# fixie-ai/ultravox

Measured on NVIDIA H100. Metric: audio-sec/s prefill (Llama-3.1-8B, 30s clip) at 1/2/4/8 H100; TTFT p50, higher is better.
Workload: dtype bf16

## Files before the change

include/uvx.h:

```cpp
#ifndef UVX_H_
#define UVX_H_

#include <stddef.h>
#include <stdint.h>

#ifdef __cplusplus
extern "C" {
#endif

#define UVX_ABI_VERSION 1

#define UVX_OK 0
#define UVX_ERR_ARG (-1)
#define UVX_ERR_CUDA (-2)
#define UVX_ERR_WS (-3)

typedef void* uvx_stream_t;

int uvx_abi_version(void);
const char* uvx_last_error(void);
int64_t uvx_launch_count(void);

size_t uvx_logmel_workspace(int64_t B, int64_t L, int n_mels);
int uvx_logmel(const float* wave, int64_t B, int64_t L, int n_mels, float* out_f32, void* out_tm,
               void* workspace, size_t workspace_bytes, uvx_stream_t stream);

int uvx_debug_mel_filters(int n_mels, float* host_dense);

int uvx_mel_to_timemajor(const float* mel, int64_t N, int n_mels, int64_t T, void* out_tm, uvx_stream_t stream);

enum { UVX_ACT_NONE = 0, UVX_ACT_GELU = 1, UVX_ACT_SWIGLU = 2 };
enum { UVX_DT_BF16 = 0, UVX_DT_F32 = 1 };
enum { UVX_TILE_PLAIN = 0, UVX_TILE_ROPE_PAIRS = 1, UVX_TILE_GATE_UP_8 = 8, UVX_TILE_GATE_UP_16 = 16 };

typedef struct uvx_gemm_args {
  const void* A;
  int64_t a_batch, a_rows, K;
  int64_t a_row_stride, a_batch_stride;
  const void* W;
  int64_t N, w_row_stride;
  void* C;
  int64_t c_row_stride, c_batch_rows, c_row_offset;
  const int32_t* c_row_map;
  const void* bias;
  const void* R;
  int64_t r_row_stride, r_batch_stride;
  float alpha;
  int32_t act;
  int32_t out_dtype;
  void* workspace;
  int64_t workspace_bytes;
  const void* norm_w;
  void* norm_out;
  float norm_eps;
  int32_t w_tiled;
  int32_t rope_cols;
  const float* rope_cos;
  const float* rope_sin;
  const int32_t* rope_positions;
  int64_t rope_rows_per_seq, rope_pos_offset;
  int32_t flags;
  int32_t w_perm;
} uvx_gemm_args;

int uvx_gemm_bf16(const uvx_gemm_args* args, uvx_stream_t stream);
int uvx_debug_gemm_override(int cfg, int splits);
int uvx_debug_gemm_stages(int n);
int uvx_debug_gemm_ws(int enable, int mode, int grid);
int uvx_debug_gemm_tma_store(int on);
int uvx_debug_gemm_times(void* dev_buf);
int uvx_debug_gemm_pf(int pf);
int uvx_debug_gemm_ws_times(void* dev_buf);
int uvx_tile_weight(const void* W, int64_t N, int64_t K, int64_t w_row_stride, int32_t R, int32_t interleave, void* out,
                    uvx_stream_t stream);
int uvx_debug_gemm_cluster(int cm, int cn);
int uvx_debug_gemm_mode(int mode);

int uvx_layernorm(const void* x, const void* w, const void* b, void* y, int64_t rows, int64_t cols,
                  int64_t x_row_stride, float eps, uvx_stream_t stream);
int uvx_rmsnorm(const void* x, const void* w, void* y, int64_t rows, int64_t cols, int64_t x_row_stride,
                int64_t group_rows, int64_t group_stride, int64_t valid_elems, float eps, uvx_stream_t stream);

typedef struct uvx_attn_args {
  const void *q, *k, *v;
  void* o;
  int64_t B, Hq, Hkv, Sq, Skv, D;
  int64_t q_rs, q_bs, k_rs, k_bs, v_rs, v_bs, o_rs, o_bs;
  const int32_t* kv_len;
  int32_t causal;
  int32_t block;
// ... 89 lines not shown
```

ultravox_b200/_lib.py:

```python
from __future__ import annotations

import ctypes as C
import os
import pathlib

_HERE = pathlib.Path(__file__).resolve().parent
LIB_PATH = _HERE / "libuvx.so"

c_i64, c_i32, c_f32, c_vp, c_sz = C.c_int64, C.c_int32, C.c_float, C.c_void_p, C.c_size_t


class GemmArgs(C.Structure):
    _fields_ = [("A", c_vp), ("a_batch", c_i64), ("a_rows", c_i64), ("K", c_i64), ("a_row_stride", c_i64),
                ("a_batch_stride", c_i64), ("W", c_vp), ("N", c_i64), ("w_row_stride", c_i64), ("C", c_vp),
                ("c_row_stride", c_i64), ("c_batch_rows", c_i64), ("c_row_offset", c_i64), ("c_row_map", c_vp),
                ("bias", c_vp), ("R", c_vp), ("r_row_stride", c_i64), ("r_batch_stride", c_i64), ("alpha", c_f32),
                ("act", c_i32), ("out_dtype", c_i32), ("workspace", c_vp), ("workspace_bytes", c_i64),
                ("norm_w", c_vp), ("norm_out", c_vp), ("norm_eps", c_f32), ("w_tiled", c_i32), ("rope_cols", c_i32),
                ("rope_cos", c_vp), ("rope_sin", c_vp), ("rope_positions", c_vp), ("rope_rows_per_seq", c_i64),
                ("rope_pos_offset", c_i64), ("flags", c_i32), ("w_perm", c_i32)]


class AttnArgs(C.Structure):
    _fields_ = [("q", c_vp), ("k", c_vp), ("v", c_vp), ("o", c_vp), ("B", c_i64), ("Hq", c_i64), ("Hkv", c_i64),
                ("Sq", c_i64), ("Skv", c_i64), ("D", c_i64), ("q_rs", c_i64), ("q_bs", c_i64), ("k_rs", c_i64),
                ("k_bs", c_i64), ("v_rs", c_i64), ("v_bs", c_i64), ("o_rs", c_i64), ("o_bs", c_i64), ("kv_len", c_vp),
                ("causal", c_i32), ("block", c_i32), ("scale", c_f32), ("lse", c_vp), ("kv_start", c_vp)]


SIGNATURES = {
    "uvx_abi_version": (C.c_int, []),
    "uvx_last_error": (C.c_char_p, []),
    "uvx_launch_count": (c_i64, []),
    "uvx_logmel_workspace": (c_sz, [c_i64, c_i64, C.c_int]),
    "uvx_logmel": (C.c_int, [c_vp, c_i64, c_i64, C.c_int, c_vp, c_vp, c_vp, c_sz, c_vp]),
    "uvx_debug_mel_filters": (C.c_int, [C.c_int, c_vp]),
    "uvx_mel_to_timemajor": (C.c_int, [c_vp, c_i64, C.c_int, c_i64, c_vp, c_vp]),
    "uvx_gemm_bf16": (C.c_int, [C.POINTER(GemmArgs), c_vp]),
    "uvx_debug_gemm_override": (C.c_int, [C.c_int, C.c_int]),
    "uvx_debug_gemm_cluster": (C.c_int, [C.c_int, C.c_int]),
    "uvx_debug_gemm_mode": (C.c_int, [C.c_int]),
    "uvx_debug_gemm_pf": (C.c_int, [C.c_int]),
    "uvx_debug_gemm_stages": (C.c_int, [C.c_int]),
    "uvx_debug_gemm_times": (C.c_int, [c_vp]),
    "uvx_debug_gemm_tma_store": (C.c_int, [C.c_int]),
    "uvx_debug_gemm_ws": (C.c_int, [C.c_int, C.c_int, C.c_int]),
    "uvx_debug_gemm_ws_times": (C.c_int, [C.c_void_p]),
    "uvx_tile_weight": (C.c_int, [c_vp, c_i64, c_i64, c_i64, c_i32, c_i32, c_vp, c_vp]),
    "uvx_layernorm": (C.c_int, [c_vp, c_vp, c_vp, c_vp, c_i64, c_i64, c_i64, c_f32, c_vp]),
    "uvx_rmsnorm": (C.c_int, [c_vp, c_vp, c_vp, c_i64, c_i64, c_i64, c_i64, c_i64, c_i64, c_f32, c_vp]),
    "uvx_attention": (C.c_int, [C.POINTER(AttnArgs), c_vp]),
    "uvx_debug_attn_tc": (C.c_int, [C.c_int]),
    "uvx_attention_enc_tc": (C.c_int, [c_vp, c_i64, c_i64, c_i64, c_i64, c_i64, c_i64, c_i64, c_vp, c_i64, c_vp, c_i32, c_f32, c_vp]),
    "uvx_rope": (C.c_int, [c_vp, c_i64, c_i64, C.c_int, C.c_int, C.c_int, c_vp, c_vp, c_vp, c_i64, c_i64, c_vp]),
    "uvx_swiglu": (C.c_int, [c_vp, c_vp, c_i64, c_i64, c_i64, C.c_int, c_vp]),
    "uvx_splice_plan": (C.c_int, [c_vp, c_vp, c_vp, c_i64, c_i64, c_i64, c_i64, c_vp, c_vp]),
    "uvx_embed_splice": (C.c_int, [c_vp, c_vp, c_i64, c_vp, c_vp, c_i64, c_i64, c_vp, c_vp]),
    "uvx_lm_head": (C.c_int, [c_vp, c_i64, c_i64, c_vp, c_i64, c_i64, c_vp, c_vp]),
    "uvx_gemv_bf16": (C.c_int, [c_vp, c_i64, c_i64, c_vp, c_i64, c_i64, c_i64, c_vp, c_i64, c_vp, c_i64, C.c_int, c_vp]),
    "uvx_kv_append": (C.c_int, [c_vp, c_i64, c_i64, c_i64, c_i64, c_vp, c_vp, c_i64, c_vp, c_i64, c_vp]),
    "uvx_gemv_fused_bf16": (C.c_int, [c_vp, c_i64, c_i64, c_vp, c_i64, c_i64, c_i64, c_vp, c_i64, c_vp, c_i64, C.c_int, c_vp, C.c_float,
                                      C.c_int, c_vp]),
    "uvx_rope_kv_append": (C.c_int, [c_vp, c_i64, c_i64, C.c_int, C.c_int, C.c_int, c_vp, c_vp, c_vp, c_vp, c_vp, c_i64, c_vp, c_vp]),
    "uvx_add_i32": (C.c_int, [c_vp, c_vp, c_i64, c_i32, c_vp]),
    "uvx_kv_write": (C.c_int, [c_vp, c_i64, c_i64, c_i64, c_i64, c_vp, c_vp, c_i64, c_i64, c_i64, c_i64, c_vp]),
    "uvx_repetition_penalty": (C.c_int, [c_vp, c_i64, c_i64, c_vp, c_i64, c_vp, c_f32, c_vp, c_vp]),
# ... 55 lines not shown
```

ultravox_b200/csrc/gemm_tc.cu:

```cuda
#include <stdlib.h>

#include "uvx_common.cuh"
#include "tc_ptx.cuh"

namespace uvx {

struct GemmParams {
  int64_t a_rows, a_batch, K, N;
  void* C;
  int64_t c_row_stride, c_batch_rows, c_row_offset;
  const int32_t* c_row_map;
  const bf16* bias;
  const bf16* R;
  int64_t r_row_stride, r_batch_stride;
  float alpha;
  int act, out_f32;
  int m_tiles;
  int n_tiles, num_tiles;
  int splits, kb_per_split;
  float* ws_partial;
  const bf16* norm_w;
  bf16* norm_out;
  float norm_eps;
  int w_tiled;
  int w_perm;
  int swiglu;
  const float* rope_cos;
  const float* rope_sin;
  const int32_t* rope_pos;
  int64_t rope_rows_per_seq, rope_pos_offset;
  int rope_cols;
  int stages;
  int cm, cn;
};

static constexpr int kSmemTotal = 227 * 1024;
static constexpr int kMaxStages = 8;
static constexpr int kGemmThreads = 384;

template <int MT, int BN>
struct WgLayout {
  static constexpr int kABytes = MT * 128 * kBK * 2;
  static constexpr int kWBytes = BN * kBK * 2;
  static constexpr int kStageBytes = kABytes + kWBytes;
  static constexpr int kRingMax = kSmemTotal - 1024 - 256;
  static constexpr int kStages = kRingMax / kStageBytes > kMaxStages ? kMaxStages : kRingMax / kStageBytes;
  static constexpr int kAcc = BN / 2;
  static_assert(kStages >= 2, "ring too shallow");
  static_assert(MT * kAcc <= 128, "accumulators must fit the register file");
};

__device__ __forceinline__ int tile_col(int tc, int perm) {
  if (!perm) return tc;
  const int q = tc >> 5, j = tc & 31;
  return j < 16 ? 16 * q + j : 64 + 16 * q + (j - 16);
}

__device__ __forceinline__ int64_t out_row(const GemmParams& p, int b, int64_t m) {
  return p.c_row_map ? (int64_t)p.c_row_map[(int64_t)b * p.a_rows + m] : (int64_t)b * p.c_batch_rows + m + p.c_row_offset;
}

template <int BN, int I>
__device__ __forceinline__ void swiglu_row(const GemmParams& p, const float* a, int h, int cq, bf16* crow, int64_t n_out0) {
#pragma unroll
  for (int j = 0; j < BN / 8; ++j) {
    if ((8 * j) % (2 * I) >= I) continue;
    const int64_t f = n_out0 + (8 * j / (2 * I)) * I + (8 * j) % (2 * I) + cq;
    if (f >= p.N / 2) continue;
// ... 6 lines not shown
      o[e] = __bfloat162float(__float2bfloat16_rn(silu_fast(gate))) * up;
    }
    *reinterpret_cast<__nv_bfloat162*>(crow + f) = __floats2bfloat162_rn(o[0], o[1]);
  }
}

__device__ __forceinline__ void rope_store(const GemmParams& p, float x1a, float x1b, float x2a, float x2b, int64_t pos, int d, bf16* crow) {
  const float2 cs = *reinterpret_cast<const float2*>(p.rope_cos + pos * 64 + d);
  const float2 sn = *reinterpret_cast<const float2*>(p.rope_sin + pos * 64 + d);
  float o1a, o2a, o1b, o2b;
  rope_pair(__bfloat162float(__float2bfloat16_rn(x1a * p.alpha)), __bfloat162float(__float2bfloat16_rn(x2a * p.alpha)), cs.x, sn.x, o1a, o2a);
  rope_pair(__bfloat162float(__float2bfloat16_rn(x1b * p.alpha)), __bfloat162float(__float2bfloat16_rn(x2b * p.alpha)), cs.y, sn.y, o1b, o2b);
  *reinterpret_cast<__nv_bfloat162*>(crow + d) = __floats2bfloat162_rn(o1a, o1b);
  *reinterpret_cast<__nv_bfloat162*>(crow + d + 64) = __floats2bfloat162_rn(o2a, o2b);
}

template <int MT, int BN>
__global__ void __launch_bounds__(kGemmThreads, 1)
gemm_wg_kernel(const __grid_constant__ CUtensorMap tmA, const __grid_constant__ CUtensorMap tmW, const GemmParams p) {
  using L = WgLayout<MT, BN>;
  pdl_trigger();
  extern __shared__ uint8_t smem_raw[];
  uint8_t* smem = (uint8_t*)(((uintptr_t)smem_raw + 1023) & ~(uintptr_t)1023);
  uint64_t* full_bar = (uint64_t*)(smem + p.stages * L::kStageBytes);
  uint64_t* empty_bar = full_bar + kMaxStages;

  const int wg = threadIdx.x >> 7, tid = threadIdx.x & 127;
  const int tiles_m_total = p.m_tiles * (int)p.a_batch;
  const int num_kb = (int)((p.K + kBK - 1) / kBK);
  const int stages = p.stages;
  const int csize = p.cm * p.cn;
  const int rank = csize > 1 ? (int)cluster_ctarank() : 0;
  const int rm = rank / p.cn, rn = rank % p.cn;
  const int cluster_tiles_m = tiles_m_total / p.cm;
  const int num_units = p.num_tiles / csize * p.splits;
  const int first_unit = blockIdx.x / csize, unit_step = gridDim.x / csize;

  if (threadIdx.x == 0) {
    for (int s = 0; s < stages; ++s) {
      mbar_init(&full_bar[s], 1);
      mbar_init(&empty_bar[s], 8 * csize);
    }
    asm volatile("fence.mbarrier_init.release.cluster;" ::: "memory");
    asm volatile("fence.proxy.async.shared::cta;" ::: "memory");
  }
  if (csize > 1) cluster_sync();
  else __syncthreads();
  pdl_wait();

  if (wg == 0) {
    asm volatile("setmaxnreg.dec.sync.aligned.u32 40;");
    if (tid == 0) {
      asm volatile("prefetch.tensormap [%0];" ::"l"(&tmA) : "memory");
      asm volatile("prefetch.tensormap [%0];" ::"l"(&tmW) : "memory");
      const int a_slice = MT * 128 / p.cn, w_slice = BN / p.cm;
      const uint16_t row_mask = (uint16_t)(((1u << p.cn) - 1u) << (rm * p.cn));
      uint16_t col_mask = 0;
      for (int j = 0; j < p.cm; ++j) col_mask |= (uint16_t)(1u << (j * p.cn + rn));
      int s = 0;
      uint32_t ph = 0;
      for (int unit = first_unit; unit < num_units; unit += unit_step) {
        const int ctile = unit / p.splits, split = unit % p.splits;
        const int tm_idx = (ctile % cluster_tiles_m) * p.cm + rm;
        const int tn_idx = (ctile / cluster_tiles_m) * p.cn + rn;
        const int b = tm_idx / p.m_tiles;
        const int m0 = (tm_idx % p.m_tiles) * (MT * 128);
        const int kb_begin = split * p.kb_per_split;
        const int kb_end = min(num_kb, kb_begin + p.kb_per_split);
        const int wt_base = tn_idx * num_kb * BN;
        for (int kb = kb_begin; kb < kb_end; ++kb) {
          mbar_wait(&empty_bar[s], ph ^ 1u);
          uint8_t* sa = smem + s * L::kStageBytes;
          mbar_expect_tx(&full_bar[s], (uint32_t)L::kStageBytes);
          uint8_t* da = sa + rn * a_slice * (kBK * 2);
          if (p.cn > 1) tma_load_3d_mc(da, &tmA, kb * kBK, m0 + rn * a_slice, b, &full_bar[s], row_mask);
          else tma_load_3d(da, &tmA, kb * kBK, m0, b, &full_bar[s]);
          uint8_t* dw = sa + L::kABytes + rm * w_slice * (kBK * 2);
          const int w0 = p.w_tiled ? 0 : kb * kBK;
          const int w1 = (p.w_tiled ? wt_base + kb * BN : tn_idx * BN) + rm * w_slice;
          if (p.cm > 1) tma_load_2d_mc(dw, &tmW, w0, w1, &full_bar[s], col_mask);
          else tma_load_2d(dw, &tmW, w0, w1, &full_bar[s]);
          if (++s == stages) { s = 0; ph ^= 1u; }
        }
      }
    }
    if (csize > 1) cluster_sync();
    return;
  }

  asm volatile("setmaxnreg.inc.sync.aligned.u32 232;");
  const int c = wg - 1;
  const int warp = tid >> 5, lane = tid & 31;
  auto release = [&](int slot) {
    __syncwarp();
    if (csize == 1) {
      if (lane == 0) mbar_arrive(&empty_bar[slot]);
    } else if (lane < csize) {
      mbar_arrive_cluster(&empty_bar[slot], (uint32_t)lane);
    }
  };
  int s = 0;
  uint32_t ph = 0;
  for (int unit = first_unit; unit < num_units; unit += unit_step) {
    const int ctile = unit / p.splits, split = unit % p.splits;
    const int tm_idx = (ctile % cluster_tiles_m) * p.cm + rm;
    const int tn_idx = (ctile / cluster_tiles_m) * p.cn + rn;
    const int b = tm_idx / p.m_tiles;
    const int m0 = (tm_idx % p.m_tiles) * (MT * 128);
    const int n0 = tn_idx * BN;
    const int kb_begin = split * p.kb_per_split;
    const int kb_end = min(num_kb, kb_begin + p.kb_per_split);

    float acc[MT][L::kAcc];
    int prev = -1;
    for (int kb = kb_begin; kb < kb_end; ++kb) {
      mbar_wait(&full_bar[s], ph);
      const uint32_t sa = smem_u32(smem + s * L::kStageBytes);
      const uint64_t dw = make_wgmma_desc(sa + L::kABytes);
      wgmma_fence();
#pragma unroll
      for (int mt = 0; mt < MT; ++mt) {
        const uint64_t da = make_wgmma_desc(sa + (mt * 128 + c * 64) * (kBK * 2));
#pragma unroll
        for (int k = 0; k < kBK / 16; ++k)
          Wgmma<BN>::mma(acc[mt], da + (uint64_t)(2 * k), dw + (uint64_t)(2 * k), (kb > kb_begin || k > 0) ? 1u : 0u);
      }
      wgmma_commit();
      wgmma_wait<1>();
      if (prev >= 0) release(prev);
      prev = s;
      if (++s == stages) { s = 0; ph ^= 1u; }
    }
    wgmma_wait<0>();
    release(prev);

    const int rq = warp * 16 + (lane >> 2);
    const int cq = 2 * (lane & 3);
    if (p.splits > 1) {
      float* part = p.ws_partial + (size_t)split * (size_t)(p.a_batch * p.a_rows) * (size_t)p.N;
#pragma unroll
      for (int mt = 0; mt < MT; ++mt) {
#pragma unroll
        for (int h = 0; h < 2; ++h) {
          const int64_t m = (int64_t)m0 + mt * 128 + c * 64 + rq + 8 * h;
          if (m >= p.a_rows) continue;
          float* dst = part + ((size_t)b * p.a_rows + m) * p.N;
#pragma unroll
          for (int j = 0; j < BN / 8; ++j) {
            const int64_t n = n0 + tile_col(8 * j + cq, p.w_perm);
            if (n < p.N) *reinterpret_cast<float2*>(dst + n) = make_float2(acc[mt][4 * j + 2 * h], acc[mt][4 * j + 2 * h + 1]);
          }
        }
      }
      continue;
    }
    if (p.swiglu) {
      const int64_t n_out0 = (int64_t)tn_idx * (BN / 2);
// ... 380 lines not shown
  CUresult r = enc(tm, CU_TENSOR_MAP_DATA_TYPE_BFLOAT16, (cuuint32_t)rank, const_cast<void*>(base), gd, gs, bx, es,
                   CU_TENSOR_MAP_INTERLEAVE_NONE, CU_TENSOR_MAP_SWIZZLE_128B, promo, CU_TENSOR_MAP_FLOAT_OOB_FILL_NONE);
  if (r != CUDA_SUCCESS) {
    set_error("cuTensorMapEncodeTiled failed with CUresult %d (rank %d dims %llu %llu stride %llu)", (int)r, rank,
              (unsigned long long)dims[0], (unsigned long long)dims[1], (unsigned long long)strides_bytes[0]);
    return UVX_ERR_CUDA;
  }
  return UVX_OK;
}

static int num_sms() {
  static int n = 0;
  if (!n) {
    int dev = 0;
    cudaGetDevice(&dev);
    cudaDeviceGetAttribute(&n, cudaDevAttrMultiProcessorCount, dev);
    if (n <= 0) n = 132;
  }
  return n;
}

static int g_gemm_stage_cap = 0;
static int g_grid_cap = 0;

static int finish_gemm(const uvx_gemm_args* a, const GemmParams& p, cudaStream_t stream) {
  const bool want_norm = a->norm_w && a->norm_out;
  if (p.splits == 1) {
    if (!want_norm) return UVX_OK;
    return uvx_rmsnorm(a->C, a->norm_w, a->norm_out, a->a_batch * a->a_rows, a->N, a->c_row_stride, 0, 0, 0, a->norm_eps, stream);
  }
  if (want_norm && !p.out_f32 && a->N <= 8192 && !a->c_row_map && a->act == UVX_ACT_NONE) {
    launch_k(splitk_reduce_rmsnorm_kernel, dim3((unsigned)(a->a_batch * a->a_rows)), dim3(256), 0, stream, p);
    return check_launch("splitk_reduce_rmsnorm_kernel");
  }
  const int64_t total = a->a_batch * a->a_rows * (a->N / 8);
  int64_t blocks = (total + 255) / 256;
  if (blocks > (int64_t)num_sms() * 8) blocks = (int64_t)num_sms() * 8;
  launch_k(splitk_reduce_kernel, dim3((unsigned)blocks), dim3(256), 0, stream, p);
  int rc = check_launch("splitk_reduce_kernel");
  if (rc || !want_norm) return rc;
  return uvx_rmsnorm(a->C, a->norm_w, a->norm_out, a->a_batch * a->a_rows, a->N, a->c_row_stride, 0, 0, 0, a->norm_eps, stream);
}

static void legal_cluster(int mt, int bn, int tiles_m_total, int n_tiles, int* cm, int* cn) {
  if (*cm < 1 || *cm > 4 || tiles_m_total % *cm != 0 || bn % (8 * *cm) != 0) *cm = 1;
  if (*cn < 1 || *cn > 4 || n_tiles % *cn != 0 || (mt * 128) % (8 * *cn) != 0) *cn = 1;
// ... 55 lines not shown
  p.R = (const bf16*)a->R;
  p.r_row_stride = a->r_row_stride;
  p.r_batch_stride = a->r_batch_stride;
  p.alpha = a->alpha;
  p.act = a->act;
  p.out_f32 = a->out_dtype == UVX_DT_F32;
  p.norm_w = (const bf16*)a->norm_w;
  p.norm_out = (bf16*)a->norm_out;
  p.norm_eps = a->norm_eps;
  p.m_tiles = m_tiles;
  p.n_tiles = n_tiles;
  p.num_tiles = p.m_tiles * (int)a->a_batch * p.n_tiles;
  p.cm = cm;
  p.cn = cn;
  const int num_kb = (int)((a->K + kBK - 1) / kBK);
  if (a->N % BN != 0) splits = 1;
  const size_t per_split = (size_t)a->a_batch * (size_t)a->a_rows * (size_t)a->N * 4;
  while (splits > 1 && (!a->workspace || per_split * (size_t)splits > (size_t)a->workspace_bytes)) --splits;
  if (splits > num_kb) splits = num_kb;
  if (splits < 1) splits = 1;
  p.kb_per_split = (num_kb + splits - 1) / splits;
  p.splits = (num_kb + p.kb_per_split - 1) / p.kb_per_split;
  p.ws_partial = (float*)a->workspace;
  p.stages = L::kStages;
  if (g_gemm_stage_cap >= 2 && p.stages > g_gemm_stage_cap) p.stages = g_gemm_stage_cap;
  const int smem = p.stages * L::kStageBytes + 1024 + 2 * kMaxStages * 8;
  static bool attr_set = false;
  if (!attr_set) {
    cudaError_t e = cudaFuncSetAttribute(gemm_wg_kernel<MT, BN>, cudaFuncAttributeMaxDynamicSharedMemorySize, kSmemTotal);
    if (e != cudaSuccess) {
      set_error("cudaFuncSetAttribute(gemm_wg_kernel<%d,%d>, smem %d): %s", MT, BN, kSmemTotal, cudaGetErrorString(e));
      return UVX_ERR_CUDA;
    }
    attr_set = true;
  }
  const int csize = cm * cn;
  const int units = p.num_tiles / csize * p.splits;
  int max_units = num_sms();
  if (csize > 1) {
    static int max_clusters[9] = {0};
    if (!max_clusters[csize]) {
      cudaLaunchConfig_t cfg = {};
      cfg.gridDim = dim3((unsigned)csize);
      cfg.blockDim = dim3(kGemmThreads);
      cfg.dynamicSmemBytes = (size_t)smem;
      cudaLaunchAttribute attr;
      attr.id = cudaLaunchAttributeClusterDimension;
      attr.val.clusterDim.x = (unsigned)csize;
      attr.val.clusterDim.y = 1;
// ... 139 lines not shown
    const int64_t total = a->a_rows * (a->N / 128) * 8;
    const int64_t blocks = (total + 255) / 256;
    launch_k(splitk_reduce_rope_kernel, dim3((unsigned)blocks), dim3(256), 0, stream, p);
    return check_launch("splitk_reduce_rope_kernel");
  }
  return finish_gemm(a, p, stream);
}

}

static int forced = -1, forced_splits = -1;

extern "C" int uvx_debug_gemm_override(int cfg, int splits) {
  forced = cfg;
  forced_splits = splits;
  return UVX_OK;
}

extern "C" int uvx_debug_gemm_stages(int n) {
  uvx::g_gemm_stage_cap = n;
  return UVX_OK;
}

extern "C" int uvx_debug_gemm_ws(int enable, int mode, int grid) {
  (void)mode;
  uvx::g_ws_enable = enable;
  uvx::g_grid_cap = grid > 0 ? grid : 0;
  return UVX_OK;
}

static int forced_cm = 0, forced_cn = 0;
static int g_cluster_enable = -1;

extern "C" int uvx_debug_gemm_cluster(int cm, int cn) {
  forced_cm = cm;
  forced_cn = cn;
  return UVX_OK;
}

extern "C" int uvx_debug_gemm_mode(int mode) { (void)mode; return UVX_OK; }
extern "C" int uvx_debug_gemm_tma_store(int on) { (void)on; return UVX_OK; }
extern "C" int uvx_debug_gemm_times(void* dev_buf) { (void)dev_buf; return UVX_OK; }
extern "C" int uvx_debug_gemm_pf(int pf) { (void)pf; return UVX_OK; }
extern "C" int uvx_debug_gemm_ws_times(void* dev_buf) { (void)dev_buf; return UVX_OK; }

static void read_forced() {
// ... 11 lines not shown
  if (rows <= 256 && batch == 1) {
    mt = rows > 128 ? 2 : 1;
    bn = N % 128 == 0 ? 128 : 64;
    if (bn == 128 && 2 * (N / 128) >= (sms * 3) / 5 && N / 128 < sms && num_kb <= 80) mt = 1;
  } else {
    mt = 1;
    const int64_t m_tiles = (rows + 127) / 128 * batch;
    if (N % 256 == 0 && m_tiles * (N / 256) >= sms && num_kb >= 32) bn = 256;
    else bn = (N % 128 == 0 && m_tiles * (N / 128) >= sms / 2) ? 128 : 64;
  }
  const int64_t tiles = ((rows + mt * 128 - 1) / (mt * 128)) * batch * ((N + bn - 1) / bn);
  int sp = 1;
  if (tiles * 2 <= sms && num_kb >= 16) {
    sp = (int)(sms / tiles);
    if (sp > num_kb / 8) sp = num_kb / 8;
    if (sp > 16) sp = 16;
    if (sp < 1) sp = 1;
  }
  *mt_out = mt;
  *bn_out = bn;
  *splits = sp;
}

static void pick_cluster(int64_t rows, int64_t batch, int mt, int* cm, int* cn) {
  *cm = *cn = 1;
  if (g_cluster_enable < 0) {
    const char* e = getenv("UVX_GEMM_CLUSTER");
    g_cluster_enable = e ? atoi(e) : 1;
  }
  if (forced_cm > 0 || forced_cn > 0) {
    *cm = forced_cm > 0 ? forced_cm : 1;
    *cn = forced_cn > 0 ? forced_cn : 1;
    return;
  }
  if (!g_cluster_enable || rows > 256 || batch != 1) return;
  if (mt == 1 && rows > 128) {
    *cm = 2;
    *cn = 2;
  }
}

extern "C" int uvx_gemm_bf16(const uvx_gemm_args* a, uvx_stream_t stream_) {
  using namespace uvx;
  cudaStream_t stream = (cudaStream_t)stream_;
  UVX_REQUIRE(a && a->A && a->W && a->C, "uvx_gemm_bf16: null pointer");
  UVX_REQUIRE(a->a_batch >= 1 && a->a_rows >= 1 && a->K >= 8 && a->N >= 64, "uvx_gemm_bf16: empty problem");
  UVX_REQUIRE(a->K % 8 == 0 && a->N % 64 == 0, "uvx_gemm_bf16: K %% 8 and N %% 64 required (K=%lld N=%lld)",
              (long long)a->K, (long long)a->N);
  UVX_REQUIRE(a->a_row_stride % 8 == 0 && a->w_row_stride % 8 == 0 && (a->a_batch == 1 || a->a_batch_stride % 8 == 0),
              "uvx_gemm_bf16: strides must be multiples of 8 elements");
  UVX_REQUIRE(((uintptr_t)a->A % 16 == 0) && ((uintptr_t)a->W % 16 == 0) && ((uintptr_t)a->C % 16 == 0),
              "uvx_gemm_bf16: 16-byte aligned bases required");
  UVX_REQUIRE(a->c_row_stride % 8 == 0 && (!a->R || (a->r_row_stride % 8 == 0 && a->r_batch_stride % 8 == 0)),
              "uvx_gemm_bf16: output / residual strides must be multiples of 8");
  UVX_REQUIRE(a->a_rows < (1ll << 31) && a->K < (1ll << 31) && a->N < (1ll << 31), "uvx_gemm_bf16: dimension too large");
  UVX_REQUIRE(!a->workspace || (uintptr_t)a->workspace % 256 == 0, "uvx_gemm_bf16: workspace must be 256-byte aligned");
  UVX_REQUIRE(!(a->norm_w && a->norm_out) || (a->out_dtype == UVX_DT_BF16 && !a->c_row_map && a->c_row_offset == 0 &&
                                              (a->a_batch == 1 || a->c_batch_rows == a->a_rows)),
              "uvx_gemm_bf16: fused RMSNorm needs a plain bf16 output");
  UVX_REQUIRE(a->w_tiled == 0 || a->w_tiled == 64 || a->w_tiled == 128 || a->w_tiled == 208 || a->w_tiled == 256,
              "uvx_gemm_bf16: w_tiled must be 64 / 128 / 208 / 256");
// ... 14 lines not shown
    if (a->a_rows <= 16) return launch_gemm_swap<16>(a, stream);
    return launch_gemm_swap<32>(a, stream);
  }
  const bool ws = forced <= 0 && forced_splits <= 0 && gemm_ws_eligible(a);
  if (ws) {
    mt = 1;
    bn = 128;
    splits = 1;
  } else if (forced > 0) {
    const int fb = forced % 1000, fm = forced / 1000;
    if (fb == 64 || fb == 128 || fb == 208 || fb == 256) {
      if (a->N % fb == 0 || fb == 208) bn = fb;
      mt = fm == 2 ? 2 : 1;
    }
  }
  if (forced_splits > 0 && !ws) splits = forced_splits;
  if (a->w_tiled) bn = (int)a->w_tiled;
  if (a->rope_cos) {
    mt = 1;
    bn = 128;
  }
  if (bn > 128) mt = 1;
  int cm, cn;
  pick_cluster(a->a_rows, a->a_batch, mt, &cm, &cn);
  switch (mt * 1000 + bn) {
    case 1064: return launch_gemm<1, 64>(a, splits, cm, cn, stream);
    case 1128: return launch_gemm<1, 128>(a, splits, cm, cn, stream);
    case 1208: return launch_gemm<1, 208>(a, splits, cm, cn, stream);
    case 1256: return launch_gemm<1, 256>(a, splits, cm, cn, stream);
    case 2064: return launch_gemm<2, 64>(a, splits, cm, cn, stream);
    case 2128: return launch_gemm<2, 128>(a, splits, cm, cn, stream);
    default: return launch_gemm<1, 64>(a, splits, cm, cn, stream);
  }
}
```

ultravox_b200/model.py:

```python
from __future__ import annotations

import dataclasses
import os
from typing import Optional

import torch
import torch.nn as nn
from transformers.modeling_outputs import CausalLMOutputWithPast

from . import ops
from .config import LossConfig, LossFunction, UltravoxConfig

FUSE_NORM = os.environ.get("UVX_FUSE_NORM", "1") != "0"
USE_TILED = os.environ.get("UVX_TILED", "1") != "0"
FUSE_ROPE = os.environ.get("UVX_FUSE_ROPE", "1") != "0"
QKV_MODE = os.environ.get("UVX_QKV_MODE", "fused")
TILED_SET = os.environ.get("UVX_TILED_SET", "gate_up")
USE_WS = os.environ.get("UVX_GEMM_WS", "0") == "1"
FUSE_SWIGLU = os.environ.get("UVX_FUSE_SWIGLU", "1") != "0"
BF16 = torch.bfloat16


class _P(nn.Module):

# ... 499 lines not shown
        enc = self.encode_audio(audio_tm, audio_lens)
        aud = self.project_audio(enc)
        B, S = input_ids.shape
        src = ops.splice_plan(audio_token_start_idx.to(dev, torch.int64).contiguous(),
                              audio_token_len.to(dev, torch.int32).contiguous(),
                              audio_batch_size.to(dev, torch.int64).reshape(-1).contiguous(), B, S, aud.shape[1])
        return ops.embed_splice(input_ids, self.language_model.model.embed_tokens.weight, aud, src)

    def llama_hidden(self, inputs_embeds: torch.Tensor, cache: Optional[KVCache] = None,
                     kv_len: Optional[torch.Tensor] = None, kv_start: Optional[torch.Tensor] = None,
                     positions: Optional[torch.Tensor] = None) -> torch.Tensor:
        lm, tc = self.language_model, self.config.text_config
        B, S, Dm = inputs_embeds.shape
        nq, nkv, hd = tc.num_attention_heads, tc.num_key_value_heads, lm.head_dim
        eps = tc.rms_norm_eps
        dev = inputs_embeds.device
        past = cache.length if cache is not None else 0
        cos, sin = self._rope_tables(past + S)
        h = inputs_embeds.view(B * S, Dm)
        x = torch.empty_like(h)
        qkv = torch.empty(B * S, (nq + 2 * nkv) * hd, dtype=BF16, device=dev)
        att = torch.empty(B * S, nq * hd, dtype=BF16, device=dev)
        ffn = tc.intermediate_size
        tiled = self._tiled_weights()
        if USE_WS and B * S > 256:
            tiled = None
        fuse_act = tiled is not None and tiled[0]["gate_up"].swiglu
        gu = None if fuse_act else torch.empty(B * S, 2 * ffn, dtype=BF16, device=dev)
        act = torch.empty(B * S, ffn, dtype=BF16, device=dev)
        rs = qkv.stride(0)
        layers = lm.model.layers
        rope = (cos, sin, positions, S, past, (nq + nkv) * hd) if (FUSE_ROPE and QKV_MODE == "fused" and hd == 128) else None
        qkv_flags = 1 if QKV_MODE == "r1" else 0
        ops.rmsnorm(h, layers[0].input_layernorm.weight, eps, out=x)
        for li, layer in enumerate(layers):
            sa, mlp = layer.self_attn, layer.mlp
            tw = tiled[li] if tiled is not None else None
            if tw is not None and tw["qkv"] is not None:
                ops.linear_tiled(x, tw["qkv"], out=qkv, rope=rope)
            else:
                ops.linear(x, sa.qkv_w, out=qkv, rope=rope, flags=qkv_flags)
            if rope is None:
                ops.rope_(qkv, nq, nkv, hd, cos, sin, rows_per_seq=S, pos_offset=past, positions=positions)
            if cache is None:
                ops.attention_fused_qkv(qkv, B, S, nq, nkv, hd, hd ** -0.5, True, kv_len, 0, out=att, kv_start=kv_start)
            else:
                kc, vc = cache.k[li], cache.v[li]
                ops.kv_write(qkv, kc, vc, B, S, past, nq, nkv, hd)
                smax = kc.shape[1]
                ops.attention(qkv.data_ptr(), kc.data_ptr(), vc.data_ptr(), att, B, nq, nkv, S, past + S, hd,
                              (rs, S * rs, nkv * hd, smax * nkv * hd, nkv * hd, smax * nkv * hd, nq * hd, S * nq * hd),
                              hd ** -0.5, True, kv_len, 0, kv_start)
            n1 = (layer.post_attention_layernorm.weight, eps, x) if FUSE_NORM else None
            if tw is not None and tw["o"] is not None:
                ops.linear_tiled(att, tw["o"], residual=h, out=h, norm=n1)
            else:
                ops.linear(att, sa.o_proj.weight, residual=h, out=h, norm=n1)
            if not FUSE_NORM:
                ops.rmsnorm(h, layer.post_attention_layernorm.weight, eps, out=x)
            if fuse_act:
                ops.linear_tiled(x, tw["gate_up"], out=act, act=ops.ACT_SWIGLU)
            else:
                if tw is not None:
                    ops.linear_tiled(x, tw["gate_up"], out=gu)
                else:
                    ops.linear(x, mlp.gate_up_w, out=gu)
                ops.swiglu(gu, gate_first=True, out=act)
            nxt = layers[li + 1].input_layernorm.weight if li + 1 < len(layers) else lm.model.norm.weight
            n2 = (nxt, eps, x) if FUSE_NORM else None
            if tw is not None and tw["down"] is not None:
                ops.linear_tiled(act, tw["down"], residual=h, out=h, norm=n2)
            else:
                ops.linear(act, mlp.down_proj.weight, residual=h, out=h, norm=n2)
            if not FUSE_NORM:
                ops.rmsnorm(h, nxt, eps, out=x)
        if cache is not None:
            cache.length = past + S
        return x.view(B, S, Dm)

    def load_state_dict(self, state_dict, strict: bool = True, _track: bool = True, **kwargs):
        import re
        from . import lora
        if lora.has_lora_keys(state_dict):
            scaling = {"audio_tower": lora.lora_scaling(getattr(self.config, "audio_model_lora_config", None)),
                       "language_model": lora.lora_scaling(getattr(self.config, "text_model_lora_config", None))}
            state_dict = lora.merge_lora_state_dict(state_dict, scaling)
        if self.language_model.tied and "language_model.lm_head.weight" not in state_dict \
                and "language_model.model.embed_tokens.weight" in state_dict:
            state_dict = dict(state_dict)
            state_dict["language_model.lm_head.weight"] = state_dict["language_model.model.embed_tokens.weight"]
        if _track:
            self.keep_params.update(state_dict.keys())
        res = super().load_state_dict(state_dict, strict=False, **kwargs)
        ignorable = [re.compile(p.replace(".", r"\.").replace("*", ".*")) for p in self._keys_to_ignore_on_load_missing]
        missing = [k for k in res.missing_keys if not any(r.match(k) for r in ignorable)]
        if strict and (missing or res.unexpected_keys):
# ... 266 lines not shown
```

ultravox_b200/ops.py:

```python
from __future__ import annotations

import ctypes as C
import math
from typing import Optional

import torch

from . import _lib
from ._lib import AttnArgs, GemmArgs, check, lib

ACT_NONE, ACT_GELU = 0, 1
BF16 = torch.bfloat16


def _stream() -> int:
    return torch.cuda.current_stream().cuda_stream


def _cuda(t: torch.Tensor, dtype=None, name="tensor") -> torch.Tensor:
    if not t.is_cuda:
        raise _lib.UvxError(f"{name} must be a CUDA tensor (ultravox_b200 has no CPU path)")
    if dtype is not None and t.dtype != dtype:
        raise TypeError(f"{name} must be {dtype}, got {t.dtype}")
    return t
# ... 17 lines not shown
    need = lib().uvx_logmel_workspace(B, L, n_mels)
    if workspace is None or workspace.numel() < need:
        workspace = torch.empty(need, dtype=torch.uint8, device=wave.device)
    check(lib().uvx_logmel(wave.data_ptr(), B, L, n_mels, _p(out_f32), _p(out_tm), workspace.data_ptr(),
                           workspace.numel(), _stream()), "uvx_logmel")
    if want_f32 and want_tm:
        return out_f32, out_tm
    return out_f32 if want_f32 else out_tm


def mel_to_timemajor(audio_values: torch.Tensor, out: Optional[torch.Tensor] = None) -> torch.Tensor:
    _cuda(audio_values, torch.float32, "audio_values")
    audio_values = audio_values.contiguous()
    N, n_mels, T = audio_values.shape
    if out is None:
        out = torch.empty(N, T + 2, n_mels, dtype=BF16, device=audio_values.device)
    check(lib().uvx_mel_to_timemajor(audio_values.data_ptr(), N, n_mels, T, out.data_ptr(), _stream()),
          "uvx_mel_to_timemajor")
    return out


_GEMM_WS: dict = {}
GEMM_WS_BYTES = 160 << 20


def gemm_workspace(device) -> torch.Tensor:
    idx = torch.device(device).index if torch.device(device).index is not None else torch.cuda.current_device()
    capturing = torch.cuda.is_current_stream_capturing()
    key = (idx, "graph") if capturing else (idx, torch.cuda.current_stream(idx).cuda_stream)
    ws = _GEMM_WS.get(key)
    if ws is None:
        with torch.cuda.device(idx):
            ws = torch.zeros(GEMM_WS_BYTES, dtype=torch.uint8, device=torch.device("cuda", idx))
            _GEMM_WS[key] = ws
            if not capturing and (idx, "graph") not in _GEMM_WS:
                _GEMM_WS[(idx, "graph")] = torch.zeros(GEMM_WS_BYTES, dtype=torch.uint8, device=torch.device("cuda", idx))
    return ws


def gemm_raw(A_ptr: int, a_batch: int, a_rows: int, K: int, a_row_stride: int, a_batch_stride: int,
             W: torch.Tensor, C_t: torch.Tensor, c_row_stride: int, c_batch_rows: int, c_row_offset: int = 0,
             c_row_map: Optional[torch.Tensor] = None, bias: Optional[torch.Tensor] = None,
             R: Optional[torch.Tensor] = None, r_row_stride: int = 0, r_batch_stride: int = 0,
             alpha: float = 1.0, act: int = ACT_NONE, norm: Optional[tuple] = None, rope: Optional[tuple] = None,
             flags: int = 0) -> None:
    a = GemmArgs()
# ... 20 lines not shown

class TiledWeight:

    def __init__(self, w: torch.Tensor, R: int, swiglu: bool = False, rope_pairs: bool = False):
        _cuda(w, BF16, "w")
        self.N, self.K, self.R, self.swiglu = int(w.shape[0]), int(w.shape[1]), int(R), bool(swiglu)
        self.rope_pairs = bool(rope_pairs)
        if rope_pairs and (swiglu or R != 128 or self.N % 128 != 0):
            raise ValueError("rope_pairs: a 128-row image of whole 128-wide heads")
        n_tiles = -(-self.N // R)
        self.image = torch.empty(n_tiles * (self.K // 64) * R * 64, dtype=BF16, device=w.device)
        inter = ((16 if R == 128 else 8) if swiglu else (1 if rope_pairs else 0))
        check(lib().uvx_tile_weight(w.data_ptr(), self.N, self.K, w.stride(0), R, inter, self.image.data_ptr(), _stream()), "uvx_tile_weight")

    @property
    def n_out(self) -> int:
        return self.N // 2 if self.swiglu else self.N


ACT_SWIGLU = 2


def linear_tiled(x: torch.Tensor, wt: TiledWeight, out: Optional[torch.Tensor] = None, residual: Optional[torch.Tensor] = None,
                 act: int = ACT_NONE, norm: Optional[tuple] = None, rope: Optional[tuple] = None) -> torch.Tensor:
    _cuda(x, BF16, "x")
    K = x.shape[-1]
    x2 = x.reshape(-1, K)
    if x2.stride(-1) != 1:
        x2 = x2.contiguous()
    M = x2.shape[0]
    n_out = wt.n_out if act == ACT_SWIGLU else wt.N
    if (act == ACT_SWIGLU) != wt.swiglu:
        raise ValueError("ACT_SWIGLU needs (and only works with) the gate|up-interleaved weight image")
    if out is None:
        out = torch.empty(*x.shape[:-1], n_out, dtype=BF16, device=x.device)
    o2 = out.view(-1, n_out)
    a = GemmArgs()
    a.A, a.a_batch, a.a_rows, a.K = x2.data_ptr(), 1, M, K
    a.a_row_stride, a.a_batch_stride = x2.stride(0), 0
    a.W, a.N, a.w_row_stride = wt.image.data_ptr(), wt.N, K
    a.C, a.c_row_stride, a.c_batch_rows, a.c_row_offset = o2.data_ptr(), o2.stride(0), M, 0
    if residual is not None:
        r2 = residual.reshape(-1, n_out)
        a.R, a.r_row_stride = r2.data_ptr(), r2.stride(0)
    a.alpha, a.act, a.out_dtype = 1.0, act, 0
    ws = gemm_workspace(out.device)
    a.workspace, a.workspace_bytes = ws.data_ptr(), ws.numel()
    if norm is not None:
        a.norm_w, a.norm_eps, a.norm_out = norm[0].data_ptr(), float(norm[1]), norm[2].data_ptr()
    a.w_tiled = wt.R
    a.w_perm = 1 if wt.rope_pairs else 0
    if rope is not None:
        cos, sin, positions, rows_per_seq, pos_offset, rope_cols = rope
        a.rope_cos, a.rope_sin, a.rope_positions = cos.data_ptr(), sin.data_ptr(), _p(positions)
        a.rope_rows_per_seq, a.rope_pos_offset, a.rope_cols = int(rows_per_seq), int(pos_offset), int(rope_cols)
    check(lib().uvx_gemm_bf16(C.byref(a), _stream()), "uvx_gemm_bf16(tiled)")
    return out


def linear(x: torch.Tensor, w: torch.Tensor, bias: Optional[torch.Tensor] = None, act: int = ACT_NONE,
# ... 404 lines not shown
```

Before: 1406.

## Split GEMM smem ring into separate A and W rings with early weight prefetch

Splits the single shared-memory stage ring into independent activation and weight rings, each with its own barriers and producer thread. The weight producer can issue TMA loads before the programmatic-dependent-launch wait, so weights stream in while the previous kernel finishes. Weights get a deeper ring for 1x128 tiles, and 2-MT single-split GEMMs now use a 1x4 cluster that multicasts A. The risk is extra barrier traffic and shallower rings under the smem budget, and issuing weight loads before the PDL wait is only safe because weights are immutable. That is why the model disables it on the call that first builds the tiled weights.

```diff
diff --git a/include/uvx.h b/include/uvx.h
--- a/include/uvx.h
+++ b/include/uvx.h
@@ -31,6 +31,7 @@
 
 enum { UVX_ACT_NONE = 0, UVX_ACT_GELU = 1, UVX_ACT_SWIGLU = 2 };
 enum { UVX_DT_BF16 = 0, UVX_DT_F32 = 1 };
+enum { UVX_GEMM_W_EARLY = 4 };
 enum { UVX_TILE_PLAIN = 0, UVX_TILE_ROPE_PAIRS = 1, UVX_TILE_GATE_UP_8 = 8, UVX_TILE_GATE_UP_16 = 16 };
 
 typedef struct uvx_gemm_args {
@@ -66,6 +67,7 @@
 int uvx_gemm_bf16(const uvx_gemm_args* args, uvx_stream_t stream);
 int uvx_debug_gemm_override(int cfg, int splits);
 int uvx_debug_gemm_stages(int n);
+int uvx_debug_gemm_ring(int a_stages, int w_stages);
 int uvx_debug_gemm_ws(int enable, int mode, int grid);
 int uvx_debug_gemm_tma_store(int on);
 int uvx_debug_gemm_times(void* dev_buf);
diff --git a/ultravox_b200/_lib.py b/ultravox_b200/_lib.py
--- a/ultravox_b200/_lib.py
+++ b/ultravox_b200/_lib.py
@@ -42,6 +42,7 @@
     "uvx_debug_gemm_mode": (C.c_int, [C.c_int]),
     "uvx_debug_gemm_pf": (C.c_int, [C.c_int]),
     "uvx_debug_gemm_stages": (C.c_int, [C.c_int]),
+    "uvx_debug_gemm_ring": (C.c_int, [C.c_int, C.c_int]),
     "uvx_debug_gemm_times": (C.c_int, [c_vp]),
     "uvx_debug_gemm_tma_store": (C.c_int, [C.c_int]),
     "uvx_debug_gemm_ws": (C.c_int, [C.c_int, C.c_int, C.c_int]),
diff --git a/ultravox_b200/csrc/gemm_tc.cu b/ultravox_b200/csrc/gemm_tc.cu
--- a/ultravox_b200/csrc/gemm_tc.cu
+++ b/ultravox_b200/csrc/gemm_tc.cu
@@ -31,11 +31,14 @@
   int64_t rope_rows_per_seq, rope_pos_offset;
   int rope_cols;
   int stages;
+  int a_stages, w_stages;
+  int w_early;
   int cm, cn;
 };
 
 static constexpr int kSmemTotal = 227 * 1024;
 static constexpr int kMaxStages = 8;
+static constexpr int kMaxRing = 16;
 static constexpr int kGemmThreads = 384;
 
 template <int MT, int BN>
@@ -43,7 +46,8 @@
   static constexpr int kABytes = MT * 128 * kBK * 2;
   static constexpr int kWBytes = BN * kBK * 2;
   static constexpr int kStageBytes = kABytes + kWBytes;
-  static constexpr int kRingMax = kSmemTotal - 1024 - 256;
+  static constexpr int kBarBytes = 4 * kMaxRing * 8;
+  static constexpr int kRingMax = kSmemTotal - 1024 - kBarBytes;
   static constexpr int kStages = kRingMax / kStageBytes > kMaxStages ? kMaxStages : kRingMax / kStageBytes;
   static constexpr int kAcc = BN / 2;
   static_assert(kStages >= 2, "ring too shallow");
@@ -96,13 +100,15 @@
   pdl_trigger();
   extern __shared__ uint8_t smem_raw[];
   uint8_t* smem = (uint8_t*)(((uintptr_t)smem_raw + 1023) & ~(uintptr_t)1023);
-  uint64_t* full_bar = (uint64_t*)(smem + p.stages * L::kStageBytes);
-  uint64_t* empty_bar = full_bar + kMaxStages;
+  uint8_t* w_ring = smem + p.a_stages * L::kABytes;
+  uint64_t* full_a = (uint64_t*)(w_ring + p.w_stages * L::kWBytes);
+  uint64_t* empty_a = full_a + kMaxRing;
+  uint64_t* full_w = empty_a + kMaxRing;
+  uint64_t* empty_w = full_w + kMaxRing;
 
   const int wg = threadIdx.x >> 7, tid = threadIdx.x & 127;
   const int tiles_m_total = p.m_tiles * (int)p.a_batch;
   const int num_kb = (int)((p.K + kBK - 1) / kBK);
-  const int stages = p.stages;
   const int csize = p.cm * p.cn;
   const int rank = csize > 1 ? (int)cluster_ctarank() : 0;
   const int rm = rank / p.cn, rn = rank % p.cn;
@@ -111,50 +117,70 @@
   const int first_unit = blockIdx.x / csize, unit_step = gridDim.x / csize;
 
   if (threadIdx.x == 0) {
-    for (int s = 0; s < stages; ++s) {
-      mbar_init(&full_bar[s], 1);
-      mbar_init(&empty_bar[s], 8 * csize);
+    for (int s = 0; s < p.a_stages; ++s) {
+      mbar_init(&full_a[s], 1);
+      mbar_init(&empty_a[s], 8 * csize);
+    }
+    for (int s = 0; s < p.w_stages; ++s) {
+      mbar_init(&full_w[s], 1);
+      mbar_init(&empty_w[s], 8 * csize);
     }
     asm volatile("fence.mbarrier_init.release.cluster;" ::: "memory");
     asm volatile("fence.proxy.async.shared::cta;" ::: "memory");
   }
   if (csize > 1) cluster_sync();
   else __syncthreads();
-  pdl_wait();
 
   if (wg == 0) {
     asm volatile("setmaxnreg.dec.sync.aligned.u32 40;");
     if (tid == 0) {
-      asm volatile("prefetch.tensormap [%0];" ::"l"(&tmA) : "memory");
       asm volatile("prefetch.tensormap [%0];" ::"l"(&tmW) : "memory");
-      const int a_slice = MT * 128 / p.cn, w_slice = BN / p.cm;
-      const uint16_t row_mask = (uint16_t)(((1u << p.cn) - 1u) << (rm * p.cn));
+      const int w_slice = BN / p.cm;
       uint16_t col_mask = 0;
       for (int j = 0; j < p.cm; ++j) col_mask |= (uint16_t)(1u << (j * p.cn + rn));
+      const int before_wait = p.w_early ? p.w_stages : 0;
+      int n = 0;
+      int s = 0;
+      uint32_t ph = 0;
+      for (int unit = first_unit; unit < num_units; unit += unit_step) {
+        const int ctile = unit / p.splits, split = unit % p.splits;
+        const int tn_idx = (ctile / cluster_tiles_m) * p.cn + rn;
+        const int kb_begin = split * p.kb_per_split;
+        const int kb_end = min(num_kb, kb_begin + p.kb_per_split);
+        const int wt_base = tn_idx * num_kb * BN;
+        for (int kb = kb_begin; kb < kb_end; ++kb) {
+          if (n++ == before_wait) pdl_wait();
+          mbar_wait(&empty_w[s], ph ^ 1u);
+          mbar_expect_tx(&full_w[s], (uint32_t)L::kWBytes);
+          uint8_t* dw = w_ring + s * L::kWBytes + rm * w_slice * (kBK * 2);
+          const int w0 = p.w_tiled ? 0 : kb * kBK;
+          const int w1 = (p.w_tiled ? wt_base + kb * BN : tn_idx * BN) + rm * w_slice;
+          if (p.cm > 1) tma_load_2d_mc(dw, &tmW, w0, w1, &full_w[s], col_mask);
+          else tma_load_2d(dw, &tmW, w0, w1, &full_w[s]);
+          if (++s == p.w_stages) { s = 0; ph ^= 1u; }
+        }
+      }
+    } else if (tid == 32) {
+      pdl_wait();
+      asm volatile("prefetch.tensormap [%0];" ::"l"(&tmA) : "memory");
+      const int a_slice = MT * 128 / p.cn;
+      const uint16_t row_mask = (uint16_t)(((1u << p.cn) - 1u) << (rm * p.cn));
       int s = 0;
       uint32_t ph = 0;
       for (int unit = first_unit; unit < num_units; unit += unit_step) {
         const int ctile = unit / p.splits, split = unit % p.splits;
         const int tm_idx = (ctile % cluster_tiles_m) * p.cm + rm;
-        const int tn_idx = (ctile / cluster_tiles_m) * p.cn + rn;
         const int b = tm_idx / p.m_tiles;
         const int m0 = (tm_idx % p.m_tiles) * (MT * 128);
         const int kb_begin = split * p.kb_per_split;
         const int kb_end = min(num_kb, kb_begin + p.kb_per_split);
-        const int wt_base = tn_idx * num_kb * BN;
         for (int kb = kb_begin; kb < kb_end; ++kb) {
-          mbar_wait(&empty_bar[s], ph ^ 1u);
-          uint8_t* sa = smem + s * L::kStageBytes;
-          mbar_expect_tx(&full_bar[s], (uint32_t)L::kStageBytes);
-          uint8_t* da = sa + rn * a_slice * (kBK * 2);
-          if (p.cn > 1) tma_load_3d_mc(da, &tmA, kb * kBK, m0 + rn * a_slice, b, &full_bar[s], row_mask);
-          else tma_load_3d(da, &tmA, kb * kBK, m0, b, &full_bar[s]);
-          uint8_t* dw = sa + L::kABytes + rm * w_slice * (kBK * 2);
-          const int w0 = p.w_tiled ? 0 : kb * kBK;
-          const int w1 = (p.w_tiled ? wt_base + kb * BN : tn_idx * BN) + rm * w_slice;
-          if (p.cm > 1) tma_load_2d_mc(dw, &tmW, w0, w1, &full_bar[s], col_mask);
-          else tma_load_2d(dw, &tmW, w0, w1, &full_bar[s]);
-          if (++s == stages) { s = 0; ph ^= 1u; }
+          mbar_wait(&empty_a[s], ph ^ 1u);
+          mbar_expect_tx(&full_a[s], (uint32_t)L::kABytes);
+          uint8_t* da = smem + s * L::kABytes + rn * a_slice * (kBK * 2);
+          if (p.cn > 1) tma_load_3d_mc(da, &tmA, kb * kBK, m0 + rn * a_slice, b, &full_a[s], row_mask);
+          else tma_load_3d(da, &tmA, kb * kBK, m0, b, &full_a[s]);
+          if (++s == p.a_stages) { s = 0; ph ^= 1u; }
         }
       }
     }
@@ -162,19 +188,24 @@
     return;
   }
 
+  pdl_wait();
   asm volatile("setmaxnreg.inc.sync.aligned.u32 232;");
   const int c = wg - 1;
   const int warp = tid >> 5, lane = tid & 31;
-  auto release = [&](int slot) {
+  auto release = [&](int a_slot, int w_slot) {
     __syncwarp();
     if (csize == 1) {
-      if (lane == 0) mbar_arrive(&empty_bar[slot]);
+      if (lane == 0) {
+        mbar_arrive(&empty_a[a_slot]);
+        mbar_arrive(&empty_w[w_slot]);
+      }
     } else if (lane < csize) {
-      mbar_arrive_cluster(&empty_bar[slot], (uint32_t)lane);
+      mbar_arrive_cluster(&empty_a[a_slot], (uint32_t)lane);
+      mbar_arrive_cluster(&empty_w[w_slot], (uint32_t)lane);
     }
   };
-  int s = 0;
-  uint32_t ph = 0;
+  int sa_i = 0, sw_i = 0;
+  uint32_t pa = 0, pw = 0;
   for (int unit = first_unit; unit < num_units; unit += unit_step) {
     const int ctile = unit / p.splits, split = unit % p.splits;
     const int tm_idx = (ctile % cluster_tiles_m) * p.cm + rm;
@@ -186,11 +217,12 @@
     const int kb_end = min(num_kb, kb_begin + p.kb_per_split);
 
     float acc[MT][L::kAcc];
-    int prev = -1;
+    int prev_a = -1, prev_w = -1;
     for (int kb = kb_begin; kb < kb_end; ++kb) {
-      mbar_wait(&full_bar[s], ph);
-      const uint32_t sa = smem_u32(smem + s * L::kStageBytes);
-      const uint64_t dw = make_wgmma_desc(sa + L::kABytes);
+      mbar_wait(&full_a[sa_i], pa);
+      mbar_wait(&full_w[sw_i], pw);
+      const uint32_t sa = smem_u32(smem + sa_i * L::kABytes);
+      const uint64_t dw = make_wgmma_desc(smem_u32(w_ring + sw_i * L::kWBytes));
       wgmma_fence();
 #pragma unroll
       for (int mt = 0; mt < MT; ++mt) {
@@ -201,12 +233,14 @@
       }
       wgmma_commit();
       wgmma_wait<1>();
-      if (prev >= 0) release(prev);
-      prev = s;
-      if (++s == stages) { s = 0; ph ^= 1u; }
+      if (prev_a >= 0) release(prev_a, prev_w);
+      prev_a = sa_i;
+      prev_w = sw_i;
+      if (++sa_i == p.a_stages) { sa_i = 0; pa ^= 1u; }
+      if (++sw_i == p.w_stages) { sw_i = 0; pw ^= 1u; }
     }
     wgmma_wait<0>();
-    release(prev);
+    release(prev_a, prev_w);
 
     const int rq = warp * 16 + (lane >> 2);
     const int cq = 2 * (lane & 3);
@@ -633,6 +667,30 @@
 
 static int g_gemm_stage_cap = 0;
 static int g_grid_cap = 0;
+static int g_ring_a = 0, g_ring_w = 0;
+
+static void ring_depths(int mt, int bn, int64_t rows, int64_t batch, int equal, int a_bytes, int w_bytes, int budget, int* a_out,
+                        int* w_out) {
+  int a = equal, w = equal;
+  if (mt == 1 && bn == 128 && (rows > 256 || batch != 1)) {
+    a = 4;
+    w = 8;
+  }
+  if (g_ring_a > 0) a = g_ring_a;
+  if (g_ring_w > 0) w = g_ring_w;
+  if (g_gemm_stage_cap >= 2) {
+    a = a < g_gemm_stage_cap ? a : g_gemm_stage_cap;
+    w = w < g_gemm_stage_cap ? w : g_gemm_stage_cap;
+  }
+  a = a < 2 ? 2 : (a > kMaxRing ? kMaxRing : a);
+  w = w < 2 ? 2 : (w > kMaxRing ? kMaxRing : w);
+  while (a * a_bytes + w * w_bytes > budget) {
+    if (w > 2) --w;
+    else --a;
+  }
+  *a_out = a;
+  *w_out = w;
+}
 
 static int finish_gemm(const uvx_gemm_args* a, const GemmParams& p, cudaStream_t stream) {
   const bool want_norm = a->norm_w && a->norm_out;
@@ -734,9 +792,9 @@
   p.kb_per_split = (num_kb + splits - 1) / splits;
   p.splits = (num_kb + p.kb_per_split - 1) / p.kb_per_split;
   p.ws_partial = (float*)a->workspace;
-  p.stages = L::kStages;
-  if (g_gemm_stage_cap >= 2 && p.stages > g_gemm_stage_cap) p.stages = g_gemm_stage_cap;
-  const int smem = p.stages * L::kStageBytes + 1024 + 2 * kMaxStages * 8;
+  ring_depths(MT, BN, a->a_rows, a->a_batch, L::kStages, L::kABytes, L::kWBytes, L::kRingMax, &p.a_stages, &p.w_stages);
+  p.w_early = (a->flags & 4) ? 1 : 0;
+  const int smem = p.a_stages * L::kABytes + p.w_stages * L::kWBytes + 1024 + L::kBarBytes;
   static bool attr_set = false;
   if (!attr_set) {
     cudaError_t e = cudaFuncSetAttribute(gemm_wg_kernel<MT, BN>, cudaFuncAttributeMaxDynamicSharedMemorySize, kSmemTotal);
@@ -922,6 +980,12 @@
   return UVX_OK;
 }
 
+extern "C" int uvx_debug_gemm_ring(int a_stages, int w_stages) {
+  uvx::g_ring_a = a_stages > 0 ? a_stages : 0;
+  uvx::g_ring_w = w_stages > 0 ? w_stages : 0;
+  return UVX_OK;
+}
+
 extern "C" int uvx_debug_gemm_ws(int enable, int mode, int grid) {
   (void)mode;
   uvx::g_ws_enable = enable;
@@ -979,7 +1043,7 @@
   *splits = sp;
 }
 
-static void pick_cluster(int64_t rows, int64_t batch, int mt, int* cm, int* cn) {
+static void pick_cluster(int64_t rows, int64_t batch, int mt, int splits, int* cm, int* cn) {
   *cm = *cn = 1;
   if (g_cluster_enable < 0) {
     const char* e = getenv("UVX_GEMM_CLUSTER");
@@ -994,6 +1058,8 @@
   if (mt == 1 && rows > 128) {
     *cm = 2;
     *cn = 2;
+  } else if (mt == 2 && splits == 1) {
+    *cn = 4;
   }
 }
 
@@ -1054,7 +1120,7 @@
   }
   if (bn > 128) mt = 1;
   int cm, cn;
-  pick_cluster(a->a_rows, a->a_batch, mt, &cm, &cn);
+  pick_cluster(a->a_rows, a->a_batch, mt, splits, &cm, &cn);
   switch (mt * 1000 + bn) {
     case 1064: return launch_gemm<1, 64>(a, splits, cm, cn, stream);
     case 1128: return launch_gemm<1, 128>(a, splits, cm, cn, stream);
diff --git a/ultravox_b200/model.py b/ultravox_b200/model.py
--- a/ultravox_b200/model.py
+++ b/ultravox_b200/model.py
@@ -545,7 +545,9 @@
         qkv = torch.empty(B * S, (nq + 2 * nkv) * hd, dtype=BF16, device=dev)
         att = torch.empty(B * S, nq * hd, dtype=BF16, device=dev)
         ffn = tc.intermediate_size
+        fresh = getattr(self, "_tiled", None) is None
         tiled = self._tiled_weights()
+        wf = 0 if fresh and self._tiled else ops.GEMM_W_EARLY
         if USE_WS and B * S > 256:
             tiled = None
         fuse_act = tiled is not None and tiled[0]["gate_up"].swiglu
@@ -560,9 +562,9 @@
             sa, mlp = layer.self_attn, layer.mlp
             tw = tiled[li] if tiled is not None else None
             if tw is not None and tw["qkv"] is not None:
-                ops.linear_tiled(x, tw["qkv"], out=qkv, rope=rope)
+                ops.linear_tiled(x, tw["qkv"], out=qkv, rope=rope, flags=wf)
             else:
-                ops.linear(x, sa.qkv_w, out=qkv, rope=rope, flags=qkv_flags)
+                ops.linear(x, sa.qkv_w, out=qkv, rope=rope, flags=qkv_flags | wf)
             if rope is None:
                 ops.rope_(qkv, nq, nkv, hd, cos, sin, rows_per_seq=S, pos_offset=past, positions=positions)
             if cache is None:
@@ -576,25 +578,25 @@
                               hd ** -0.5, True, kv_len, 0, kv_start)
             n1 = (layer.post_attention_layernorm.weight, eps, x) if FUSE_NORM else None
             if tw is not None and tw["o"] is not None:
-                ops.linear_tiled(att, tw["o"], residual=h, out=h, norm=n1)
+                ops.linear_tiled(att, tw["o"], residual=h, out=h, norm=n1, flags=wf)
             else:
-                ops.linear(att, sa.o_proj.weight, residual=h, out=h, norm=n1)
+                ops.linear(att, sa.o_proj.weight, residual=h, out=h, norm=n1, flags=wf)
             if not FUSE_NORM:
                 ops.rmsnorm(h, layer.post_attention_layernorm.weight, eps, out=x)
             if fuse_act:
-                ops.linear_tiled(x, tw["gate_up"], out=act, act=ops.ACT_SWIGLU)
+                ops.linear_tiled(x, tw["gate_up"], out=act, act=ops.ACT_SWIGLU, flags=wf)
             else:
                 if tw is not None:
-                    ops.linear_tiled(x, tw["gate_up"], out=gu)
+                    ops.linear_tiled(x, tw["gate_up"], out=gu, flags=wf)
                 else:
-                    ops.linear(x, mlp.gate_up_w, out=gu)
+                    ops.linear(x, mlp.gate_up_w, out=gu, flags=wf)
                 ops.swiglu(gu, gate_first=True, out=act)
             nxt = layers[li + 1].input_layernorm.weight if li + 1 < len(layers) else lm.model.norm.weight
             n2 = (nxt, eps, x) if FUSE_NORM else None
             if tw is not None and tw["down"] is not None:
-                ops.linear_tiled(act, tw["down"], residual=h, out=h, norm=n2)
+                ops.linear_tiled(act, tw["down"], residual=h, out=h, norm=n2, flags=wf)
             else:
-                ops.linear(act, mlp.down_proj.weight, residual=h, out=h, norm=n2)
+                ops.linear(act, mlp.down_proj.weight, residual=h, out=h, norm=n2, flags=wf)
             if not FUSE_NORM:
                 ops.rmsnorm(h, nxt, eps, out=x)
         if cache is not None:
diff --git a/ultravox_b200/ops.py b/ultravox_b200/ops.py
--- a/ultravox_b200/ops.py
+++ b/ultravox_b200/ops.py
@@ -63,6 +63,7 @@
 
 _GEMM_WS: dict = {}
 GEMM_WS_BYTES = 160 << 20
+GEMM_W_EARLY = 4
 
 
 def gemm_workspace(device) -> torch.Tensor:
@@ -129,7 +130,7 @@
 
 
 def linear_tiled(x: torch.Tensor, wt: TiledWeight, out: Optional[torch.Tensor] = None, residual: Optional[torch.Tensor] = None,
-                 act: int = ACT_NONE, norm: Optional[tuple] = None, rope: Optional[tuple] = None) -> torch.Tensor:
+                 act: int = ACT_NONE, norm: Optional[tuple] = None, rope: Optional[tuple] = None, flags: int = 0) -> torch.Tensor:
     _cuda(x, BF16, "x")
     K = x.shape[-1]
     x2 = x.reshape(-1, K)
@@ -143,6 +144,7 @@
         out = torch.empty(*x.shape[:-1], n_out, dtype=BF16, device=x.device)
     o2 = out.view(-1, n_out)
     a = GemmArgs()
+    a.flags = flags
     a.A, a.a_batch, a.a_rows, a.K = x2.data_ptr(), 1, M, K
     a.a_row_stride, a.a_batch_stride = x2.stride(0), 0
     a.W, a.N, a.w_row_stride = wt.image.data_ptr(), wt.N, K
```

Result: faster. 1433, median of 6 (+1.9%).
